# tqch/v-diffusion-torch

Hardware: AMD Instinct MI355X
Metric: train_images_per_sec (higher is better)
Workload: dtype fp32 (bf16x3 split products in the tile-engine GEMMs)

## Files before the change

### v-diffusion-torch_amd/csrc/wino43.hip

```cpp
#include "common.h"
#include "../../include/vdiff_hip_dgrad_planes.h"
#include <stdlib.h>
#include <type_traits>

namespace {

typedef __attribute__((address_space(3))) void* lds_ptr_t;
constexpr unsigned OOB = 0x80000000u;
constexpr int KT = 8;
constexpr int TN = 32;
constexpr int TILES = 64;
constexpr int U_STAGE = 36 * 4 * 16 * 2 * 2;
constexpr int THREADS = 512;

struct Args43 {
    const float* x; long long ldx;
    const float* U;
    float* y; long long ldy;
    int nimg, H, W, K, N;
    int items_per_img;
    int ngrp;
    int ncb, nitems;
    const float* bias; const float* res; long long ldr;
    float* stats;
// ... 527 lines not shown
        }
    } else {
        if (c4 >= p.Cout) return;
        f32x4 R[4][6];
#pragma unroll
        for (int u = 0; u < 4; ++u) {
            f32x4 y[4];
#pragma unroll
            for (int v = 0; v < 4; ++v)
                y[v] = *reinterpret_cast<const f32x4*>(p.dy + ((long long)(img * p.H + 4 * ty + u) * p.W + 4 * tx + v) * p.lddy + c4);
            a6(y, R[u]);
        }
#pragma unroll
        for (int b = 0; b < 6; ++b) {
            const f32x4 col[4] = {R[0][b], R[1][b], R[2][b], R[3][b]};
            f32x4 o[6];
            a6(col, o);
#pragma unroll
            for (int a = 0; a < 6; ++a)
                st_once(p.dM + ((long long)((tile >> 4) * 36 + 6 * a + b) * 16 + (tile & 15)) * p.Cout + c4, o[a]);
        }
    }
}

__global__ __launch_bounds__(256) void wino43_wgrad_finish_kernel(const float* dU, const float* cs, int Cout, int Cin, int Cout_w, int Cin_w,
                                                                  float* dw, float* dbias, int accumulate) {
    const long long idx = (long long)blockIdx.x * blockDim.x + threadIdx.x;
    if (dbias && idx < Cout_w) {
        const double pv[6] = {-1.0 / 9, 8.0 / 9, 0.0, 2.0 / 9, 0.0, -1.0 / 8};
        double c = 0.0;
#pragma unroll
        for (int a = 0; a < 6; ++a)
#pragma unroll
            for (int b = 0; b < 6; ++b)
                if (pv[a] != 0.0 && pv[b] != 0.0) c += pv[a] * pv[b] * (double)cs[(long long)(6 * a + b) * Cout + idx];
        dbias[idx] = accumulate ? dbias[idx] + (float)c : (float)c;
    }
    if (idx >= (long long)Cout * Cin) return;
    const int co = (int)(idx / Cin), ci = (int)(idx - (long long)co * Cin);
    if (co >= Cout_w || ci >= Cin_w) return;
    float u[6][6];
#pragma unroll
    for (int a = 0; a < 6; ++a)
#pragma unroll
        for (int b = 0; b < 6; ++b) u[a][b] = dU[(long long)(6 * a + b) * Cout * Cin + idx];
    constexpr float g0 = 64.f / 81, g12 = 128.f / 243, g34 = 32.f / 243, h12 = 32.f / 81, h34 = 16.f / 81, k = 8.f / 27;
    float t[3][6];
#pragma unroll
    for (int b = 0; b < 6; ++b) {
        const float s12 = u[1][b] + u[2][b], d12 = u[2][b] - u[1][b], s34 = u[3][b] + u[4][b], d34 = u[3][b] - u[4][b];
        t[0][b] = g0 * u[0][b] - g12 * s12 + g34 * s34;
        t[1][b] = h12 * d12 + h34 * d34;
        t[2][b] = k * (s34 - s12) + u[5][b];
    }
    float* o = dw + ((long long)co * Cin_w + ci) * 9;
#pragma unroll
    for (int r = 0; r < 3; ++r) {
        const float s12 = t[r][1] + t[r][2], d12 = t[r][2] - t[r][1], s34 = t[r][3] + t[r][4], d34 = t[r][3] - t[r][4];
        const float w0 = g0 * t[r][0] - g12 * s12 + g34 * s34;
        const float w1 = h12 * d12 + h34 * d34;
        const float w2 = k * (s34 - s12) + t[r][5];
        o[3 * r] = accumulate ? o[3 * r] + w0 : w0;
        o[3 * r + 1] = accumulate ? o[3 * r + 1] + w1 : w1;
        o[3 * r + 2] = accumulate ? o[3 * r + 2] + w2 : w2;
    }
}

constexpr long long FUSED_FINISH_MIN = 147456;
__global__ __launch_bounds__(384) void wino43_wgrad_reduce_finish_kernel(const float* slabs, const float* cpart, int S, int Cout, int Cin,
                                                                         int Cout_w, int Cin_w, float* dw, float* dbias, int accumulate) {
    __shared__ float tsh[3][6][64];
    const int x = threadIdx.x, b = threadIdx.y;
    const long long idx = (long long)blockIdx.x * 64 + x;
    if (dbias && b == 0 && idx < Cout_w) {
        const double pv[6] = {-1.0 / 9, 8.0 / 9, 0.0, 2.0 / 9, 0.0, -1.0 / 8};
        double c = 0.0;
#pragma unroll
        for (int a = 0; a < 6; ++a)
#pragma unroll
            for (int bb = 0; bb < 6; ++bb)
                if (pv[a] != 0.0 && pv[bb] != 0.0) {
                    float cs = 0.f;
                    for (int z = 0; z < S; ++z) cs += cpart[((long long)(6 * a + bb) * S + z) * Cout + idx];
                    c += pv[a] * pv[bb] * (double)cs;
                }
        dbias[idx] = accumulate ? dbias[idx] + (float)c : (float)c;
    }
    const long long plane = (long long)Cout * Cin;
    const bool in = idx < plane;
    constexpr float g0 = 64.f / 81, g12 = 128.f / 243, g34 = 32.f / 243, h12 = 32.f / 81, h34 = 16.f / 81, k = 8.f / 27;
    {
        float u[6] = {0.f, 0.f, 0.f, 0.f, 0.f, 0.f};
        if (in) {
            const float* sl = slabs + (long long)b * S * plane + idx;
            const long long astep = 6LL * S * plane;
            for (int z = 0; z < S; ++z) {
#pragma unroll
                for (int a = 0; a < 6; ++a) u[a] += sl[a * astep + z * plane];
            }
        }
        const float s12 = u[1] + u[2], d12 = u[2] - u[1], s34 = u[3] + u[4], d34 = u[3] - u[4];
        tsh[0][b][x] = g0 * u[0] - g12 * s12 + g34 * s34;
        tsh[1][b][x] = h12 * d12 + h34 * d34;
        tsh[2][b][x] = k * (s34 - s12) + u[5];
    }
    __syncthreads();
    if (!in || b >= 3) return;
    const int co = (int)(idx / Cin), ci = (int)(idx - (long long)co * Cin);
    if (co >= Cout_w || ci >= Cin_w) return;
    const int r = b;
    float t[6];
#pragma unroll
    for (int c = 0; c < 6; ++c) t[c] = tsh[r][c][x];
    const float s12 = t[1] + t[2], d12 = t[2] - t[1], s34 = t[3] + t[4], d34 = t[3] - t[4];
    const float w0 = g0 * t[0] - g12 * s12 + g34 * s34;
    const float w1 = h12 * d12 + h34 * d34;
    const float w2 = k * (s34 - s12) + t[5];
    float* o = dw + ((long long)co * Cin_w + ci) * 9 + 3 * r;
    o[0] = accumulate ? o[0] + w0 : w0;
    o[1] = accumulate ? o[1] + w1 : w1;
    o[2] = accumulate ? o[2] + w2 : w2;
}

__device__ __forceinline__ void pack43_planes(const float* src, float* dst, long long plane) {
    const double Gd[6][3] = {{64.0 / 81, 0.0, 0.0}, {-128.0 / 243, -32.0 / 81, -8.0 / 27}, {-128.0 / 243, 32.0 / 81, -8.0 / 27},
                             {32.0 / 243, 16.0 / 81, 8.0 / 27}, {32.0 / 243, -16.0 / 81, 8.0 / 27}, {0.0, 0.0, 1.0}};
    double g[3][3], tmp[6][3];
#pragma unroll
    for (int a = 0; a < 3; ++a)
#pragma unroll
        for (int b = 0; b < 3; ++b) g[a][b] = (double)src[a * 3 + b];
#pragma unroll
    for (int a = 0; a < 6; ++a)
#pragma unroll
        for (int c = 0; c < 3; ++c) tmp[a][c] = Gd[a][0] * g[0][c] + Gd[a][1] * g[1][c] + Gd[a][2] * g[2][c];
#pragma unroll
    for (int a = 0; a < 6; ++a)
#pragma unroll
        for (int b = 0; b < 6; ++b) dst[(6 * a + b) * plane] = (float)(tmp[a][0] * Gd[b][0] + tmp[a][1] * Gd[b][1] + tmp[a][2] * Gd[b][2]);
}

__global__ __launch_bounds__(256) void wino43_pack_planes_kernel(const float* w, float* U, int Cout, int Cin) {
    const long long idx = (long long)blockIdx.x * 256 + threadIdx.x, plane = (long long)Cout * Cin;
    if (idx >= plane) return;
    pack43_planes(w + idx * 9, U + idx, plane);
}

__global__ __launch_bounds__(256) void wino43_pack_planes_t_kernel(const float* w, float* Ut, int Cout, int Cin) {
    const long long idx = (long long)blockIdx.x * 256 + threadIdx.x, plane = (long long)Cout * Cin;
    if (idx >= plane) return;
    const long long ci = idx / Cout, co = idx - ci * Cout;
    pack43_planes(w + (co * Cin + ci) * 9, Ut + idx, plane);
}

__device__ __forceinline__ void at4(const f32x4 (&m)[6], f32x4 (&o)[4]) {
    const f32x4 p12 = m[1] + m[2], q12 = m[1] - m[2], p34 = m[3] + m[4], q34 = m[3] - m[4];
    o[0] = m[0] + p12 + p34;
    o[1] = 0.75f * q12 + 1.5f * q34;
    o[2] = 0.5625f * p12 + 2.25f * p34;
    o[3] = 0.421875f * q12 + 3.375f * q34 + m[5];
}

struct Out43 {
    const float* M; long long plane;
    const float* bias; const float* res; long long ldr;
    float* y; long long ldy;
    float* stats;
    int H, W, Cout, TW, TPI, T, CT;
};

__global__ __launch_bounds__(256) void wino43_out_transform_kernel(const Out43 p) {
    __shared__ float ssum[2][16][64];
    const int q = threadIdx.x, tl = threadIdx.y;
    const int c4 = blockIdx.y * 64 + 4 * q;
    const bool in = c4 < p.Cout;
    f32x4 s1 = {0.f, 0.f, 0.f, 0.f}, s2 = s1;
    if (in) {
        f32x4 bv = {0.f, 0.f, 0.f, 0.f};
        if (p.bias) bv = *reinterpret_cast<const f32x4*>(p.bias + c4);
        for (int i = 0; i < p.CT; i += 16) {
            const int tile = blockIdx.x * p.CT + i + tl;
            if (tile >= p.T) break;
            const int img = tile / p.TPI, tin = tile - img * p.TPI;
            const int ty = tin / p.TW, tx = tin - ty * p.TW;
            const float* mp = p.M + (long long)tile * p.Cout + c4;
            f32x4 S[6][4];
#pragma unroll
            for (int a = 0; a < 6; ++a) {
                f32x4 m[6];
#pragma unroll
                for (int b = 0; b < 6; ++b) m[b] = *reinterpret_cast<const f32x4*>(mp + (long long)(6 * a + b) * p.plane);
                at4(m, S[a]);
            }
            const long long pix0 = ((long long)img * p.H + 4 * ty) * p.W + 4 * tx;
#pragma unroll
            for (int v = 0; v < 4; ++v) {
                const f32x4 col[6] = {S[0][v], S[1][v], S[2][v], S[3][v], S[4][v], S[5][v]};
                f32x4 o[4];
                at4(col, o);
#pragma unroll
                for (int u = 0; u < 4; ++u) {
                    const long long pix = pix0 + (long long)u * p.W + v;
                    f32x4 val = o[u] + bv;
                    if (p.res) val += *reinterpret_cast<const f32x4*>(p.res + pix * p.ldr + c4);
                    s1 += val; s2 += val * val;
                    *reinterpret_cast<f32x4*>(p.y + pix * p.ldy + c4) = val;
                }
            }
        }
    }
    if (!p.stats) return;
#pragma unroll
    for (int j = 0; j < 4; ++j) { ssum[0][tl][4 * q + j] = s1[j]; ssum[1][tl][4 * q + j] = s2[j]; }
    __syncthreads();
    const int tid = tl * 16 + q;
    if (tid < 128) {
        const int st = tid >> 6, ch = tid & 63;
        if (blockIdx.y * 64 + ch < p.Cout) {
            float v = 0.f;
#pragma unroll
            for (int k = 0; k < 16; ++k) v += ssum[st][k][ch];
            p.stats[((long long)blockIdx.x * 2 + st) * p.Cout + blockIdx.y * 64 + ch] = v;
        }
    }
}

__device__ __forceinline__ void b6(const f32x4 (&v)[6], f32x4 (&o)[6]) {
    const f32x4 p12 = v[1] + v[2], q12 = v[2] - v[1], p34 = v[3] + v[4], q34 = v[4] - v[3];
    o[0] = 1.265625f * v[0];
    o[1] = 1.6875f * q12 + 0.84375f * q34 + 1.265625f * v[5];
    o[2] = -2.8125f * v[0] - 2.25f * p12 - 0.5625f * p34;
    o[3] = -0.75f * q12 - 1.5f * q34 - 2.8125f * v[5];
    o[4] = v[0] + p12 + p34;
    o[5] = v[5];
}

struct In43 {
    const float* dV; long long plane;
    float* dx; long long lddx;
    int Cin;
};

template <int TW>
__global__ __launch_bounds__(256) void wino43_in_transpose_kernel(const In43 p) {
    constexpr int TPI = TW * TW, NQ = 256 / TPI;
    __shared__ f32x4 ring[12][256];
    const int tid = threadIdx.x, q = tid % NQ, tile = tid / NQ;
    const int ty = tile / TW, tx = tile - ty * TW;
    const int c4 = ((int)blockIdx.x * NQ + q) * 4;
    const bool in = c4 < p.Cin;
    f32x4 S[6][4];
    if (in) {
        const float* vp = p.dV + ((long long)blockIdx.y * TPI + tile) * p.Cin + c4;
#pragma unroll
        for (int a = 0; a < 6; ++a) {
            f32x4 v[6], r[6];
#pragma unroll
            for (int b = 0; b < 6; ++b) v[b] = *reinterpret_cast<const f32x4*>(vp + (long long)(6 * a + b) * p.plane);
            b6(v, r);
            ring[a][tid] = r[0]; ring[6 + a][tid] = r[5];
#pragma unroll
            for (int c = 0; c < 4; ++c) S[a][c] = r[c + 1];
        }
    }
    __syncthreads();
    if (in) {
        if (tx > 0) {
#pragma unroll
            for (int a = 0; a < 6; ++a) S[a][0] += ring[6 + a][tid - NQ];
        }
        if (tx < TW - 1) {
#pragma unroll
            for (int a = 0; a < 6; ++a) S[a][3] += ring[a][tid + NQ];
        }
    }
    __syncthreads();
    f32x4 P[4][4];
    if (in) {
#pragma unroll
        for (int c = 0; c < 4; ++c) {
            const f32x4 col[6] = {S[0][c], S[1][c], S[2][c], S[3][c], S[4][c], S[5][c]};
            f32x4 o[6];
            b6(col, o);
            ring[c][tid] = o[0]; ring[4 + c][tid] = o[5];
#pragma unroll
            for (int u = 0; u < 4; ++u) P[u][c] = o[u + 1];
        }
    }
    __syncthreads();
    if (!in) return;
    if (ty > 0) {
#pragma unroll
        for (int c = 0; c < 4; ++c) P[0][c] += ring[4 + c][tid - TW * NQ];
    }
    if (ty < TW - 1) {
#pragma unroll
        for (int c = 0; c < 4; ++c) P[3][c] += ring[c][tid + TW * NQ];
    }
    float* xp = p.dx + (((long long)blockIdx.y * (4 * TW) + 4 * ty) * (4 * TW) + 4 * tx) * p.lddx + c4;
#pragma unroll
    for (int u = 0; u < 4; ++u)
#pragma unroll
        for (int c = 0; c < 4; ++c) *reinterpret_cast<f32x4*>(xp + (long long)(u * 4 * TW + c) * p.lddx) = P[u][c];
}

struct Wg43Plan { bool ok; int T, S; size_t v_f, m_f, u_f, cs_f, gemm_bytes; };
Wg43Plan wg43_plan(int nimg, int H, int W, int Cin, int Cout) {
    Wg43Plan g = {};
    if (nimg <= 0 || H % 4 || W % 4 || H < 4 || W < 4 || Cin % 4 || Cout % 4) return g;
    g.T = nimg * (H / 4) * (W / 4);
    g.S = vd_gemm_grouped_wgrad_auto_split(36, Cout, Cin, g.T, (g.T + 1535) / 1536, 24);
    const size_t T16 = ((size_t)g.T + 15) / 16 * 16;
    g.v_f = (size_t)36 * T16 * Cin; g.m_f = (size_t)36 * T16 * Cout; g.u_f = (size_t)36 * Cout * Cin; g.cs_f = (size_t)36 * Cout;
    g.gemm_bytes = vd_gemm_grouped_wgrad_ws_bytes(36, Cout, Cin, g.S);
    g.ok = true;
    return g;
}

#ifndef VD_PLANES_MIN_TILES
#define VD_PLANES_MIN_TILES 8192
#endif
#ifndef VD_PLANES_TRAINING
#define VD_PLANES_TRAINING 1
#endif
#ifndef VD_PLANES_INFERENCE
#define VD_PLANES_INFERENCE 0
#endif
thread_local int g_last43 = 0;
#ifdef VD_PROBES
unsigned long long* g_probe43 = nullptr;
#else
constexpr unsigned long long* g_probe43 = nullptr;
#endif
thread_local int g_last43w = 0;

}

extern "C" int vd_conv3x3_dgrad_wino43_supported(int32_t nimg, int32_t H, int32_t W, int32_t Cin, int32_t Cout, int64_t lddy, int64_t lddx) {
    if (nimg <= 0 || Cout % KT || Cin % TN || lddy % 4 || lddx % 4) return 0;
    if (!((W == 32 && H == 32) || (W == 64 && H % 16 == 0 && H >= 16) || (W == 16 && H == 16 && nimg % 4 == 0))) return 0;
    const long long px = (W == 16 ? (long long)nimg : 1LL) * H * W, lim = 0x7FFFFFF0LL / 4;
    if (px * lddy >= lim || px * lddx >= lim) return 0;
    return 1;
}

extern "C" size_t vd_wino43_u_floats(int32_t Cout, int32_t Cin) { return (size_t)36 * Cout * Cin; }

extern "C" int vd_conv3x3_wino43_preferred(int32_t nimg, int32_t H, int32_t W, int32_t N) {
    if (nimg <= 0 || N <= 0) return 0;
    const long long grp = W == 16 ? (nimg + 3) / 4 : (long long)nimg * (W == 64 ? H / 16 : 1);
    const long long i43 = grp * ((N + TN - 1) / TN), ncu = vd_persistent_cus();
    const long long r43 = (i43 + ncu - 1) / ncu, r23 = (4 * i43 + ncu - 1) / ncu;
    return 8 * r43 < 3 * r23;
}

extern "C" int vd_conv3x3_dgrad_wino43(const float* dy, int64_t lddy, const float* U43, float* dx, int64_t lddx, int32_t nimg, int32_t H,
                                       int32_t W, int32_t Cin, int32_t Cout, void* stream) {
    VD_REQUIRE(dy && U43 && dx, "vd_conv3x3_dgrad_wino43: null operand");
    VD_REQUIRE(vd_conv3x3_dgrad_wino43_supported(nimg, H, W, Cin, Cout, lddy, lddx),
               "vd_conv3x3_dgrad_wino43: unsupported geometry nimg=%d H=%d W=%d Cin=%d Cout=%d", nimg, H, W, Cin, Cout);
    VD_REQUIRE(vd_aligned16(dy) && vd_aligned16(U43) && vd_aligned16(dx), "vd_conv3x3_dgrad_wino43: operands must be 16-byte aligned");
    Args43 a = {};
    a.x = dy; a.ldx = lddy; a.U = U43; a.y = dx; a.ldy = lddx;
    a.nimg = nimg; a.H = H; a.W = W; a.K = Cout; a.N = Cin;
    a.items_per_img = W == 64 ? H / 16 : 1;
    a.ngrp = W == 16 ? nimg / 4 : nimg * a.items_per_img;
    a.ncb = Cin / TN;
    const long long items = (long long)a.ngrp * a.ncb;
    VD_REQUIRE(items < (1LL << 30), "vd_conv3x3_dgrad_wino43: too many work items");
    a.nitems = (int)items;
    a.probe = g_probe43;
    const int ncu = vd_persistent_cus();
    const dim3 grid((unsigned)(items < ncu ? items : ncu)), blk(THREADS);
    hipStream_t st = (hipStream_t)stream;
    if (W == 16) hipLaunchKernelGGL((wino43_conv_kernel<4, false>), grid, blk, 0, st, a);
    else if (W == 32) hipLaunchKernelGGL((wino43_conv_kernel<8, false>), grid, blk, 0, st, a);
    else hipLaunchKernelGGL((wino43_conv_kernel<16, false>), grid, blk, 0, st, a);
    VD_LAUNCH_CHECK("wino43_conv_kernel<., false>");
    g_last43 = W / 4;
    return 0;
}

extern "C" int vd_wino43_last_kernel(void) { return g_last43; }
#ifdef VD_PROBES
extern "C" int vd_wino43_set_probe(unsigned long long* buf) { g_probe43 = buf; return 0; }
#endif

extern "C" int vd_wino43_pack(const float* w_oihw, int32_t Cout, int32_t Cin, float* U43, void* stream) {
    VD_REQUIRE(w_oihw && U43 && Cout % KT == 0 && Cin % TN == 0, "vd_wino43_pack: needs Cout %% 8 == 0 and Cin %% 32 == 0");
    hipLaunchKernelGGL(wino43_pack_kernel, dim3((unsigned)((Cin / TN) * (Cout / KT))), dim3(256), 0, (hipStream_t)stream, w_oihw, U43, Cout, Cin, 0);
    VD_LAUNCH_CHECK("wino43_pack_kernel");
    return 0;
}

extern "C" int vd_conv3x3_wino43_fwd_supported(int32_t nimg, int32_t H, int32_t W, int32_t Cin, int32_t Cout, int64_t ldx, int64_t ldy,
                                               int64_t ldres) {
    if (nimg <= 0 || Cin % KT || Cout % TN || ldx % 4 || ldy % 4 || ldres % 4) return 0;
    if (!((W == 32 && H == 32) || (W == 64 && H % 16 == 0 && H >= 16) || (W == 16 && H == 16 && nimg % 4 == 0))) return 0;
    const long long px = (W == 16 ? (long long)nimg : 1LL) * H * W, lim = 0x7FFFFFF0LL / 4;
    if (px * ldx >= lim || px * ldy >= lim || (ldres > 0 && px * ldres >= lim)) return 0;
    return 1;
}

extern "C" int vd_wino43_pack_fwd(const float* w_oihw, int32_t Cout, int32_t Cin, float* U43f, void* stream) {
    VD_REQUIRE(w_oihw && U43f && Cin % KT == 0 && Cout % TN == 0, "vd_wino43_pack_fwd: needs Cin %% 8 == 0 and Cout %% 32 == 0");
    hipLaunchKernelGGL(wino43_pack_kernel, dim3((unsigned)((Cout / TN) * (Cin / KT))), dim3(256), 0, (hipStream_t)stream, w_oihw, U43f, Cout, Cin, 1);
    VD_LAUNCH_CHECK("wino43_pack_kernel(fwd)");
    return 0;
}

extern "C" int vd_conv3x3_wino43_fwd_chunk_rows(int32_t H, int32_t W) { return W == 16 ? H * W : (W == 32 ? H * W : 16 * W); }

extern "C" int vd_conv3x3_wino43_fwd(const float* xin, int64_t ldx, const float* U43f, const float* bias, const float* res, int64_t ldres,
                                     float* y, int64_t ldy, int32_t nimg, int32_t H, int32_t W, int32_t Cin, int32_t Cout,
                                     float* stats_part, void* stream) {
    VD_REQUIRE(xin && U43f && y, "vd_conv3x3_wino43_fwd: null operand");
    VD_REQUIRE(vd_conv3x3_wino43_fwd_supported(nimg, H, W, Cin, Cout, ldx, ldy, res ? ldres : 0),
               "vd_conv3x3_wino43_fwd: unsupported geometry nimg=%d H=%d W=%d Cin=%d Cout=%d", nimg, H, W, Cin, Cout);
    VD_REQUIRE(vd_aligned16(xin) && vd_aligned16(U43f) && vd_aligned16(y) && (!res || vd_aligned16(res)) && (!bias || vd_aligned16(bias)),
               "vd_conv3x3_wino43_fwd: operands must be 16-byte aligned");
    Args43 a = {};
    a.x = xin; a.ldx = ldx; a.U = U43f; a.y = y; a.ldy = ldy;
    a.nimg = nimg; a.H = H; a.W = W; a.K = Cin; a.N = Cout;
    a.items_per_img = W == 64 ? H / 16 : 1;
    a.ngrp = W == 16 ? nimg / 4 : nimg * a.items_per_img;
    a.ncb = Cout / TN;
    a.bias = bias; a.res = res; a.ldr = ldres; a.stats = stats_part;
    a.chunks_per_img = (H * W) / vd_conv3x3_wino43_fwd_chunk_rows(H, W);
    VD_REQUIRE(a.chunks_per_img == a.items_per_img, "vd_conv3x3_wino43_fwd: statistics chunks (%d per image) do not match the work items (%d)", a.chunks_per_img, a.items_per_img);
    const long long items = (long long)a.ngrp * a.ncb;
    VD_REQUIRE(items < (1LL << 30), "vd_conv3x3_wino43_fwd: too many work items");
    a.nitems = (int)items;
    a.probe = g_probe43;
    const int ncu = vd_persistent_cus();
    const dim3 grid((unsigned)(items < ncu ? items : ncu)), blk(THREADS);
    hipStream_t st = (hipStream_t)stream;
    if (W == 16) hipLaunchKernelGGL((wino43_conv_kernel<4, true>), grid, blk, 0, st, a);
    else if (W == 32) hipLaunchKernelGGL((wino43_conv_kernel<8, true>), grid, blk, 0, st, a);
    else hipLaunchKernelGGL((wino43_conv_kernel<16, true>), grid, blk, 0, st, a);
    VD_LAUNCH_CHECK("wino43_conv_kernel<., true>");
    g_last43 = -(W / 4);
    return 0;
}

extern "C" int vd_wino43_pack_batched(const int64_t* items_dev, int32_t n, int64_t total_blocks, void* stream) {
    VD_REQUIRE(items_dev && n > 0 && total_blocks > 0 && total_blocks < (1LL << 31), "vd_wino43_pack_batched: bad table");
    hipLaunchKernelGGL(wino43_pack_batched_kernel, dim3((unsigned)total_blocks), dim3(256), 0, (hipStream_t)stream,
                       reinterpret_cast<const long long*>(items_dev), n);
    VD_LAUNCH_CHECK("wino43_pack_batched_kernel");
    return 0;
}

extern "C" int vd_conv3x3_wgrad_wino43_supported(int32_t nimg, int32_t H, int32_t W, int32_t Cin, int32_t Cout, int64_t ldx, int64_t lddy) {
    const Wg43Plan g = wg43_plan(nimg, H, W, Cin, Cout);
    if (!g.ok || ldx % 4 || lddy % 4 || g.T < 512 || g.T % 4) return 0;
    const long long px = (long long)nimg * H * W, lim = 0x7FFFFFF0LL / 4;
    if (px * ldx >= lim || px * lddy >= lim) return 0;
    if ((long long)g.T * (Cin > Cout ? Cin : Cout) * 4 >= (1LL << 40)) return 0;
    return 1;
}

extern "C" size_t vd_conv3x3_wgrad_wino43_ws_bytes(int32_t nimg, int32_t H, int32_t W, int32_t Cin, int32_t Cout) {
    const Wg43Plan g = wg43_plan(nimg, H, W, Cin, Cout);
    if (!g.ok) return 0;
    return (g.v_f + g.m_f + g.u_f + g.cs_f) * sizeof(float) + g.gemm_bytes;
}

static int wgrad43_impl(const float* xin, int64_t ldx, const float* dy, int64_t lddy, int32_t nimg, int32_t H, int32_t W, int32_t Cin,
                        int32_t Cout, float* dw_oihw, float* dbias, int32_t Cin_w, int32_t Cout_w, int32_t accumulate, float* ws,
                        size_t ws_bytes, void* stream, int phases, const float* Vgiven = nullptr, const float* dMgiven = nullptr) {
    VD_REQUIRE((xin || Vgiven) && (dy || dMgiven) && dw_oihw && ws, "vd_conv3x3_wgrad_wino43: null operand");
    VD_REQUIRE(!dMgiven || (Vgiven && !(phases & 1)), "vd_conv3x3_wgrad_wino43: a given dM needs a given V and runs no transform pass");
    VD_REQUIRE((!Vgiven || vd_aligned16(Vgiven)) && (!dMgiven || vd_aligned16(dMgiven)), "vd_conv3x3_wgrad_wino43: V / dM must be 16-byte aligned");
    VD_REQUIRE(vd_conv3x3_wgrad_wino43_supported(nimg, H, W, Cin, Cout, ldx, lddy),
               "vd_conv3x3_wgrad_wino43: unsupported geometry nimg=%d H=%d W=%d Cin=%d Cout=%d", nimg, H, W, Cin, Cout);
    VD_REQUIRE(Cin_w <= Cin && Cout_w <= Cout, "vd_conv3x3_wgrad_wino43: real dims exceed padded dims");
    VD_REQUIRE((!xin || vd_aligned16(xin)) && vd_aligned16(dy) && vd_aligned16(ws), "vd_conv3x3_wgrad_wino43: operands must be 16-byte aligned");
    VD_REQUIRE(ws_bytes >= vd_conv3x3_wgrad_wino43_ws_bytes(nimg, H, W, Cin, Cout), "vd_conv3x3_wgrad_wino43: workspace too small");
    const Wg43Plan g = wg43_plan(nimg, H, W, Cin, Cout);
    const float* V = Vgiven ? Vgiven : ws;
    float* dM = ws + g.v_f;
    float* dU = dM + g.m_f;
    float* cs = dU + g.u_f;
    float* gws = cs + g.cs_f;
    hipStream_t st = (hipStream_t)stream;
    if (phases & 1) {
        WgT43 t = {};
        t.x = xin; t.ldx = ldx; t.dy = dy; t.lddy = lddy; t.V = ws; t.dM = dM;
        t.nimg = nimg; t.H = H; t.W = W; t.Cin = Cin; t.Cout = Cout; t.TW = W / 4; t.TPI = (H / 4) * (W / 4); t.T = g.T;
        t.z0 = Vgiven ? 1 : 0;
        const int cmax = Vgiven ? Cout : (Cin > Cout ? Cin : Cout);
        hipLaunchKernelGGL(wino43_wgrad_transform_kernel, dim3((unsigned)(g.T / 4), (unsigned)((cmax + 255) / 256), Vgiven ? 1 : 2), dim3(64, 4), 0, st, t);
        VD_LAUNCH_CHECK("wino43_wgrad_transform_kernel");
    }
    if (phases & 2) {
        const float* A[36]; const float* B[36]; float* C[36]; float* colsum[36];
        for (int e = 0; e < 36; ++e) {
            A[e] = (dMgiven ? dMgiven : dM) + (size_t)e * 16 * Cout; B[e] = V + (size_t)e * 16 * Cin;
            C[e] = dU + (size_t)e * Cout * Cin; colsum[e] = cs + (size_t)e * Cout;
        }
        const int rc = vd_gemm_grouped_wgrad_kblk(A, B, C, colsum, 36, Cout, Cin, g.T, Cout, Cin, Cin, g.S, gws, g.gemm_bytes, stream,
                                                  36LL * 16 * Cout, 36LL * 16 * Cin,
                                                  (long long)Cout * Cin >= FUSED_FINISH_MIN ? 1 : 0);
        if (rc) return rc;
        g_last43w = g.S;
    }
    if (phases & 4) {
        const long long tot = (long long)Cout * Cin;
        if (tot >= FUSED_FINISH_MIN) {
            const int used = vd_gemm_grouped_wgrad_used_slabs(36, Cout, Cin, g.T, g.S);
            hipLaunchKernelGGL(wino43_wgrad_reduce_finish_kernel, dim3((unsigned)((tot + 63) / 64)), dim3(64, 6), 0, st, gws,
                               gws + (size_t)36 * used * Cout * Cin, used, Cout, Cin, Cout_w, Cin_w, dw_oihw, dbias, accumulate);
        } else {
            hipLaunchKernelGGL(wino43_wgrad_finish_kernel, dim3((unsigned)((tot + 255) / 256)), dim3(256), 0, st, dU, cs, Cout, Cin, Cout_w, Cin_w,
                               dw_oihw, dbias, accumulate);
        }
        VD_LAUNCH_CHECK("wino43_wgrad_finish_kernel");
    }
    return 0;
}

extern "C" int vd_conv3x3_wgrad_wino43(const float* xin, int64_t ldx, const float* dy, int64_t lddy, int32_t nimg, int32_t H, int32_t W,
                                       int32_t Cin, int32_t Cout, float* dw_oihw, float* dbias, int32_t Cin_w, int32_t Cout_w,
                                       int32_t accumulate, float* ws, size_t ws_bytes, void* stream) {
    return wgrad43_impl(xin, ldx, dy, lddy, nimg, H, W, Cin, Cout, dw_oihw, dbias, Cin_w, Cout_w, accumulate, ws, ws_bytes, stream, 7);
}

extern "C" int vd_conv3x3_wgrad_wino43_phase(const float* xin, int64_t ldx, const float* dy, int64_t lddy, int32_t nimg, int32_t H,
                                             int32_t W, int32_t Cin, int32_t Cout, float* dw_oihw, float* dbias, int32_t Cin_w,
                                             int32_t Cout_w, int32_t accumulate, float* ws, size_t ws_bytes, int32_t phase, void* stream) {
    VD_REQUIRE(phase == 1 || phase == 2 || phase == 4, "vd_conv3x3_wgrad_wino43_phase: phase must be 1 (transforms), 2 (GEMMs) or 4 (reduction + finish)");
    return wgrad43_impl(xin, ldx, dy, lddy, nimg, H, W, Cin, Cout, dw_oihw, dbias, Cin_w, Cout_w, accumulate, ws, ws_bytes, stream, phase);
}

extern "C" int vd_wino43_wgrad_last_kernel(void) { return g_last43w; }

extern "C" int vd_conv3x3_wgrad_wino43_v(const float* V, const float* dy, int64_t lddy, int32_t nimg, int32_t H, int32_t W, int32_t Cin,
                                         int32_t Cout, float* dw_oihw, float* dbias, int32_t Cin_w, int32_t Cout_w, int32_t accumulate,
                                         float* ws, size_t ws_bytes, int32_t phase, void* stream) {
    VD_REQUIRE(V, "vd_conv3x3_wgrad_wino43_v: null V");
    VD_REQUIRE(phase == 7 || phase == 1 || phase == 2 || phase == 4, "vd_conv3x3_wgrad_wino43_v: phase must be 7, 1, 2 or 4");
    return wgrad43_impl(nullptr, Cin, dy, lddy, nimg, H, W, Cin, Cout, dw_oihw, dbias, Cin_w, Cout_w, accumulate, ws, ws_bytes, stream, phase, V);
}

extern "C" int vd_conv3x3_wino43_fwd_planes_supported(int32_t nimg, int32_t H, int32_t W, int32_t Cin, int32_t Cout, int64_t ldx, int64_t ldy,
                                                      int64_t ldres) {
    if (nimg <= 0 || Cin <= 0 || Cout <= 0 || Cin % 4 || Cout % 4 || ldx % 4 || ldy % 4 || ldres % 4) return 0;
    if (!((W == 32 && H == 32) || (W == 64 && H % 16 == 0 && H >= 16) || (W == 16 && H == 16))) return 0;
    const long long T = (long long)nimg * (H / 4) * (W / 4);
    if (T >= (1LL << 22) || 36LL * 16 * Cin * 16 + 16LL * Cin + 256 >= 0x70000000LL / 4) return 0;
    if (128LL * Cin + 128 >= 0x70000000LL / 4 || 128LL * Cout + 128 >= 0x70000000LL / 4) return 0;
    return 1;
}

extern "C" size_t vd_conv3x3_wino43_v_floats(int32_t nimg, int32_t H, int32_t W, int32_t Cin) {
    return (size_t)36 * ((size_t)nimg * (H / 4) * (W / 4)) * Cin;
}

extern "C" size_t vd_conv3x3_wino43_fwd_planes_ws_bytes(int32_t nimg, int32_t H, int32_t W, int32_t Cin, int32_t Cout) {
    const size_t T = (size_t)nimg * (H / 4) * (W / 4);
    return ((size_t)36 * Cout * Cin + (size_t)36 * T * Cout) * sizeof(float);
}

extern "C" int vd_conv3x3_fwd_planes_preferred(int32_t nimg, int32_t H, int32_t W, int32_t Cin, int32_t Cout, int32_t training) {
    if (!vd_conv3x3_wino43_fwd_planes_supported(nimg, H, W, Cin, Cout, Cin, Cout, Cout)) return 0;
    const long long T = (long long)nimg * (H / 4) * (W / 4);
    static const long long floor_t = getenv("VD_PLANES_MIN_TILES") ? atoll(getenv("VD_PLANES_MIN_TILES")) : VD_PLANES_MIN_TILES;
    static const int inference = getenv("VD_PLANES_INFERENCE") ? atoi(getenv("VD_PLANES_INFERENCE")) : VD_PLANES_INFERENCE;
    if (T < floor_t || Cout % 256 || Cin % 16) return 0;
    return training ? VD_PLANES_TRAINING : (inference != 0);
}

extern "C" int vd_conv3x3_wino43_fwd_planes(const float* xin, int64_t ldx, const float* w_oihw, const float* bias, const float* res,
                                            int64_t ldres, float* y, int64_t ldy, int32_t nimg, int32_t H, int32_t W, int32_t Cin,
                                            int32_t Cout, float* stats_part, float* V, float* ws, size_t ws_bytes, int32_t phase, void* stream) {
    VD_REQUIRE(xin && w_oihw && y && V && ws, "vd_conv3x3_wino43_fwd_planes: null operand");
    VD_REQUIRE(vd_conv3x3_wino43_fwd_planes_supported(nimg, H, W, Cin, Cout, ldx, ldy, res ? ldres : 0),
               "vd_conv3x3_wino43_fwd_planes: unsupported geometry nimg=%d H=%d W=%d Cin=%d Cout=%d", nimg, H, W, Cin, Cout);
    VD_REQUIRE(vd_aligned16(xin) && vd_aligned16(y) && vd_aligned16(V) && vd_aligned16(ws) && (!res || vd_aligned16(res)) &&
               (!bias || vd_aligned16(bias)), "vd_conv3x3_wino43_fwd_planes: operands must be 16-byte aligned");
    VD_REQUIRE(ws_bytes >= vd_conv3x3_wino43_fwd_planes_ws_bytes(nimg, H, W, Cin, Cout), "vd_conv3x3_wino43_fwd_planes: workspace too small");
    VD_REQUIRE(phase == 7 || phase == 1 || phase == 2 || phase == 4, "vd_conv3x3_wino43_fwd_planes: phase must be 7, 1, 2 or 4");
    const int TPI = (H / 4) * (W / 4), T = nimg * TPI;
    float* Up = ws;
    float* Mb = ws + (size_t)36 * Cout * Cin;
    hipStream_t st = (hipStream_t)stream;
    if (phase & 1) {
        const long long plane = (long long)Cout * Cin;
        hipLaunchKernelGGL(wino43_pack_planes_kernel, dim3((unsigned)((plane + 255) / 256)), dim3(256), 0, st, w_oihw, Up, Cout, Cin);
        VD_LAUNCH_CHECK("wino43_pack_planes_kernel");
        WgT43 t = {};
        t.x = xin; t.ldx = ldx; t.V = V;
        t.nimg = nimg; t.H = H; t.W = W; t.Cin = Cin; t.Cout = Cout; t.TW = W / 4; t.TPI = TPI; t.T = T;
        t.z0 = 0;
        hipLaunchKernelGGL(wino43_wgrad_transform_kernel, dim3((unsigned)(T / 4), (unsigned)((Cin + 255) / 256), 1), dim3(64, 4), 0, st, t);
        VD_LAUNCH_CHECK("wino43_wgrad_transform_kernel(V)");
    }
    if (phase & 2) {
        vd_gemm_desc d = {};
        d.A = V; d.B = Up; d.C = Mb;
        d.M = T; d.N = Cout; d.K = Cin; d.a_kind = VD_ROW; d.b_kind = VD_ROW;
        d.lda = Cin; d.ldb = Cin; d.ldc = Cout;
        d.batch = 36; d.nh = 1; d.alpha = 1.f;
        d.sAb = 16LL * Cin; d.sBb = (long long)Cout * Cin; d.sCb = (long long)T * Cout;
        const int rc = vd_gemm_rowblk(&d, 36LL * 16 * Cin, stream);
        if (rc) return rc;
    }
    if (phase & 4) {
        Out43 o = {};
        o.M = Mb; o.plane = (long long)T * Cout; o.bias = bias; o.res = res; o.ldr = ldres; o.y = y; o.ldy = ldy; o.stats = stats_part;
        o.H = H; o.W = W; o.Cout = Cout; o.TW = W / 4; o.TPI = TPI; o.T = T;
        o.CT = vd_conv3x3_wino43_fwd_chunk_rows(H, W) / 16;
        hipLaunchKernelGGL(wino43_out_transform_kernel, dim3((unsigned)(T / o.CT), (unsigned)((Cout + 63) / 64)), dim3(16, 16), 0, st, o);
        VD_LAUNCH_CHECK("wino43_out_transform_kernel");
    }
    return 0;
}

extern "C" size_t vd_conv3x3_wino43_dm_floats(int32_t nimg, int32_t H, int32_t W, int32_t Cout) {
    const size_t T = (size_t)nimg * (H / 4) * (W / 4);
    return (size_t)36 * ((T + 15) / 16 * 16) * Cout;
}

extern "C" int vd_conv3x3_wino43_dy_image(const float* dy, int64_t lddy, int32_t nimg, int32_t H, int32_t W, int32_t Cout, float* dM,
                                          void* stream) {
    VD_REQUIRE(dy && dM, "vd_conv3x3_wino43_dy_image: null operand");
    VD_REQUIRE(nimg > 0 && H >= 4 && W >= 4 && H % 4 == 0 && W % 4 == 0 && Cout > 0 && Cout % 4 == 0 && lddy % 4 == 0 && lddy >= Cout,
               "vd_conv3x3_wino43_dy_image: unsupported geometry nimg=%d H=%d W=%d Cout=%d", nimg, H, W, Cout);
    VD_REQUIRE(vd_aligned16(dy) && vd_aligned16(dM), "vd_conv3x3_wino43_dy_image: operands must be 16-byte aligned");
    const long long TPI = (long long)(H / 4) * (W / 4), T = nimg * TPI;
    VD_REQUIRE(T % 4 == 0 && T < (1LL << 31) && (long long)nimg * H * W * lddy < 0x7FFFFFF0LL / 4 && T * Cout * 4 < (1LL << 40),
               "vd_conv3x3_wino43_dy_image: tile count or tensor size out of range");
    WgT43 t = {};
    t.dy = dy; t.lddy = lddy; t.dM = dM;
    t.nimg = nimg; t.H = H; t.W = W; t.Cin = Cout; t.Cout = Cout; t.TW = W / 4; t.TPI = (int)TPI; t.T = (int)T;
    t.z0 = 1;
    hipLaunchKernelGGL(wino43_wgrad_transform_kernel, dim3((unsigned)(T / 4), (unsigned)((Cout + 255) / 256), 1), dim3(64, 4), 0,
                       (hipStream_t)stream, t);
    VD_LAUNCH_CHECK("wino43_wgrad_transform_kernel(dM)");
    return 0;
}

extern "C" int vd_conv3x3_wgrad_wino43_vm(const float* V, const float* dM, int32_t nimg, int32_t H, int32_t W, int32_t Cin, int32_t Cout,
                                          float* dw_oihw, float* dbias, int32_t Cin_w, int32_t Cout_w, int32_t accumulate, float* ws,
                                          size_t ws_bytes, int32_t phase, void* stream) {
    VD_REQUIRE(V && dM, "vd_conv3x3_wgrad_wino43_vm: null V or dM");
    VD_REQUIRE(phase == 7 || phase == 2 || phase == 4, "vd_conv3x3_wgrad_wino43_vm: phase must be 7, 2 or 4");
    return wgrad43_impl(nullptr, Cin, nullptr, Cout, nimg, H, W, Cin, Cout, dw_oihw, dbias, Cin_w, Cout_w, accumulate, ws, ws_bytes, stream,
                        phase & 6, V, dM);
}

extern "C" int vd_conv3x3_wino43_dgrad_planes_supported(int32_t nimg, int32_t H, int32_t W, int32_t Cin, int32_t Cout, int64_t lddx) {
    if (nimg <= 0 || nimg > 65535 || Cin <= 0 || Cout <= 0 || Cin % 4 || Cout % 4 || lddx % 4 || lddx < Cin) return 0;
    if (!((W == 32 && H == 32) || (W == 16 && H == 16))) return 0;
    const long long T = (long long)nimg * (H / 4) * (W / 4);
    if (T >= (1LL << 22) || 36LL * 16 * Cout * 16 + 16LL * Cout + 256 >= 0x70000000LL / 4) return 0;
    if (128LL * Cin + 128 >= 0x70000000LL / 4 || 128LL * Cout + 128 >= 0x70000000LL / 4) return 0;
    return 1;
}

extern "C" size_t vd_conv3x3_wino43_dgrad_planes_ws_bytes(int32_t nimg, int32_t H, int32_t W, int32_t Cin, int32_t Cout) {
    const size_t T = (size_t)nimg * (H / 4) * (W / 4);
    return ((size_t)36 * Cout * Cin + (size_t)36 * T * Cin) * sizeof(float);
}

extern "C" int vd_conv3x3_dgrad_planes_preferred(int32_t nimg, int32_t H, int32_t W, int32_t Cin, int32_t Cout, int32_t training) {
    if (!training || !vd_conv3x3_wino43_dgrad_planes_supported(nimg, H, W, Cin, Cout, Cin)) return 0;
    static const long long floor_t = getenv("VD_PLANES_MIN_TILES") ? atoll(getenv("VD_PLANES_MIN_TILES")) : VD_PLANES_MIN_TILES;
    const long long T = (long long)nimg * (H / 4) * (W / 4);
    return T >= floor_t && Cin % 256 == 0 && Cout % 16 == 0;
}

extern "C" int vd_conv3x3_wino43_dgrad_planes(const float* dM, const float* w_oihw, float* dx, int64_t lddx, int32_t nimg, int32_t H, int32_t W,
                                              int32_t Cin, int32_t Cout, float* ws, size_t ws_bytes, int32_t phase, void* stream) {
    VD_REQUIRE(dM && w_oihw && dx && ws, "vd_conv3x3_wino43_dgrad_planes: null operand");
    VD_REQUIRE(vd_conv3x3_wino43_dgrad_planes_supported(nimg, H, W, Cin, Cout, lddx),
               "vd_conv3x3_wino43_dgrad_planes: unsupported geometry nimg=%d H=%d W=%d Cin=%d Cout=%d", nimg, H, W, Cin, Cout);
    VD_REQUIRE(vd_aligned16(dM) && vd_aligned16(dx) && vd_aligned16(ws), "vd_conv3x3_wino43_dgrad_planes: operands must be 16-byte aligned");
    VD_REQUIRE(ws_bytes >= vd_conv3x3_wino43_dgrad_planes_ws_bytes(nimg, H, W, Cin, Cout), "vd_conv3x3_wino43_dgrad_planes: workspace too small");
    VD_REQUIRE(phase == 7 || phase == 1 || phase == 2 || phase == 4, "vd_conv3x3_wino43_dgrad_planes: phase must be 7, 1, 2 or 4");
    const int TPI = (H / 4) * (W / 4), T = nimg * TPI;
    float* Ut = ws;
    float* dV = ws + (size_t)36 * Cout * Cin;
    hipStream_t st = (hipStream_t)stream;
    if (phase & 1) {
        const long long plane = (long long)Cout * Cin;
        hipLaunchKernelGGL(wino43_pack_planes_t_kernel, dim3((unsigned)((plane + 255) / 256)), dim3(256), 0, st, w_oihw, Ut, Cout, Cin);
        VD_LAUNCH_CHECK("wino43_pack_planes_t_kernel");
    }
    if (phase & 2) {
        vd_gemm_desc d = {};
        d.A = dM; d.B = Ut; d.C = dV;
        d.M = T; d.N = Cin; d.K = Cout; d.a_kind = VD_ROW; d.b_kind = VD_ROW;
        d.lda = Cout; d.ldb = Cout; d.ldc = Cin;
        d.batch = 36; d.nh = 1; d.alpha = 1.f;
        d.sAb = 16LL * Cout; d.sBb = (long long)Cout * Cin; d.sCb = (long long)T * Cin;
        const int rc = vd_gemm_rowblk(&d, 36LL * 16 * Cout, stream);
        if (rc) return rc;
    }
    if (phase & 4) {
        In43 o = {};
        o.dV = dV; o.plane = (long long)T * Cin; o.dx = dx; o.lddx = lddx; o.Cin = Cin;
        if (W == 32)
            hipLaunchKernelGGL(wino43_in_transpose_kernel<8>, dim3((unsigned)((Cin + 15) / 16), (unsigned)nimg), dim3(256), 0, st, o);
        else
            hipLaunchKernelGGL(wino43_in_transpose_kernel<4>, dim3((unsigned)((Cin + 63) / 64), (unsigned)nimg), dim3(256), 0, st, o);
        VD_LAUNCH_CHECK("wino43_in_transpose_kernel");
    }
    return 0;
}
```

Before: 2364.

## Add row-streaming Winograd F(4,3) dgrad input-transform kernel for W=32

Adds a new inverse-transform kernel for the 32-wide dgrad path. Each thread walks down the tile rows, carrying the overlapping output rows between iterations in registers (keep/down) and prefetching the next row's 36 planes with nontemporal loads while the current row is computed. A double-buffered LDS ring is used only for the horizontal neighbour exchange. It is enabled by default behind an env switch and offset-range checks. The aim is fewer overlapping-edge LDS round trips, better load/compute overlap and uniform-base addressing, at the cost of heavy register use (36+ f32x4 live) and only 128-thread blocks.

```diff
diff --git a/v-diffusion-torch_amd/csrc/wino43.hip b/v-diffusion-torch_amd/csrc/wino43.hip
--- a/v-diffusion-torch_amd/csrc/wino43.hip
+++ b/v-diffusion-torch_amd/csrc/wino43.hip
@@ -853,6 +853,91 @@
     for (int u = 0; u < 4; ++u)
 #pragma unroll
         for (int c = 0; c < 4; ++c) *reinterpret_cast<f32x4*>(xp + (long long)(u * 4 * TW + c) * p.lddx) = P[u][c];
+}
+
+__device__ __forceinline__ f32x4 add_rn(const f32x4 a, const f32x4 b) {
+#pragma clang fp contract(off)
+    return a + b;
+}
+
+__device__ __forceinline__ unsigned long long uniform64(const void* p) {
+    const unsigned long long a = reinterpret_cast<unsigned long long>(p);
+    const unsigned lo = __builtin_amdgcn_readfirstlane((unsigned)a), hi = __builtin_amdgcn_readfirstlane((unsigned)(a >> 32));
+    return ((unsigned long long)hi << 32) | lo;
+}
+typedef __attribute__((address_space(1))) char gchar;
+typedef __attribute__((address_space(1))) f32x4 gf32x4;
+__device__ __forceinline__ f32x4 ld_nt(const float* base, unsigned off) {
+    return __builtin_nontemporal_load(reinterpret_cast<const gf32x4*>(reinterpret_cast<const gchar*>(uniform64(base)) + off));
+}
+__device__ __forceinline__ void st_at(float* base, unsigned off, const f32x4 v) {
+    *reinterpret_cast<gf32x4*>(reinterpret_cast<gchar*>(uniform64(base)) + off) = v;
+}
+
+__global__ __launch_bounds__(128) void wino43_in_transpose_rows_kernel(const In43 p) {
+    constexpr int TW = 8, NQ = 16;
+    __shared__ f32x4 ring[2][12][TW * NQ];
+    const int tid = threadIdx.x, q = tid % NQ, tx = tid / NQ;
+    const bool in = (int)blockIdx.x * (4 * NQ) + 4 * q < p.Cin;
+    const float* vb = p.dV + (long long)blockIdx.y * (TW * TW) * p.Cin + (long long)blockIdx.x * (4 * NQ);
+    float* xb = p.dx + (long long)blockIdx.y * (16 * TW * TW) * p.lddx + (long long)blockIdx.x * (4 * NQ);
+    const unsigned vo = 4u * ((unsigned)tx * (unsigned)p.Cin + 4u * q), xo = 4u * (4u * tx * (unsigned)p.lddx + 4u * q);
+    f32x4 v[36], keep[4], down[4];
+    if (in) {
+#pragma unroll
+        for (int k = 0; k < 36; ++k) v[k] = ld_nt(vb + k * p.plane, vo);
+    }
+#pragma unroll 1
+    for (int ty = 0; ty < TW; ++ty) {
+        f32x4 (*rg)[TW * NQ] = ring[ty & 1];
+        f32x4 S[6][4];
+        if (in) {
+#pragma unroll
+            for (int a = 0; a < 6; ++a) {
+                const f32x4 row[6] = {v[6 * a], v[6 * a + 1], v[6 * a + 2], v[6 * a + 3], v[6 * a + 4], v[6 * a + 5]};
+                f32x4 r[6];
+                b6(row, r);
+                rg[a][tid] = r[0]; rg[6 + a][tid] = r[5];
+#pragma unroll
+                for (int c = 0; c < 4; ++c) S[a][c] = r[c + 1];
+            }
+            if (ty < TW - 1) {
+                const float* vn = vb + (long long)(ty + 1) * TW * p.Cin;
+#pragma unroll
+                for (int k = 0; k < 36; ++k) v[k] = ld_nt(vn + k * p.plane, vo);
+            }
+        }
+        __syncthreads();
+        if (in) {
+            if (tx > 0) {
+#pragma unroll
+                for (int a = 0; a < 6; ++a) S[a][0] += rg[6 + a][tid - NQ];
+            }
+            if (tx < TW - 1) {
+#pragma unroll
+                for (int a = 0; a < 6; ++a) S[a][3] += rg[a][tid + NQ];
+            }
+            float* xr = xb + (long long)ty * (16 * TW) * p.lddx;
+#pragma unroll
+            for (int c = 0; c < 4; ++c) {
+                const f32x4 col[6] = {S[0][c], S[1][c], S[2][c], S[3][c], S[4][c], S[5][c]};
+                f32x4 o[6];
+                b6(col, o);
+                if (ty > 0) {
+                    st_at(xr + (long long)(c - 4 * TW) * p.lddx, xo, add_rn(keep[c], o[0]));
+                    o[1] = add_rn(o[1], down[c]);
+                }
+#pragma unroll
+                for (int u = 0; u < 3; ++u) st_at(xr + (long long)(u * 4 * TW + c) * p.lddx, xo, o[u + 1]);
+                keep[c] = o[4]; down[c] = o[5];
+            }
+        }
+    }
+    if (in) {
+        float* xr = xb + (long long)(4 * TW - 1) * (4 * TW) * p.lddx;
+#pragma unroll
+        for (int c = 0; c < 4; ++c) st_at(xr + (long long)c * p.lddx, xo, keep[c]);
+    }
 }
 
 struct Wg43Plan { bool ok; int T, S; size_t v_f, m_f, u_f, cs_f, gemm_bytes; };
@@ -1252,7 +1337,10 @@
     if (phase & 4) {
         In43 o = {};
         o.dV = dV; o.plane = (long long)T * Cin; o.dx = dx; o.lddx = lddx; o.Cin = Cin;
-        if (W == 32)
+        static const bool rows = !(getenv("VD_DGRAD_FOLD") && atoi(getenv("VD_DGRAD_FOLD")) == 0);
+        if (W == 32 && rows && 7LL * Cin + 64 < (1LL << 30) && 28LL * lddx + 64 < (1LL << 30))
+            hipLaunchKernelGGL(wino43_in_transpose_rows_kernel, dim3((unsigned)((Cin + 63) / 64), (unsigned)nimg), dim3(128), 0, st, o);
+        else if (W == 32)
             hipLaunchKernelGGL(wino43_in_transpose_kernel<8>, dim3((unsigned)((Cin + 15) / 16), (unsigned)nimg), dim3(256), 0, st, o);
         else
             hipLaunchKernelGGL(wino43_in_transpose_kernel<4>, dim3((unsigned)((Cin + 63) / 64), (unsigned)nimg), dim3(256), 0, st, o);
```

Result: no change. 2348 (-0.7%).
